# TejasPote/data_diet_distributed

Measured on AMD Instinct MI355X. Metric: examples scored/sec (whole node), EL2N+GraNd ResNet-18 CIFAR-10, 1/2/4/8 GPU, higher is better.
Workload: dtype fp32 (split MFMA: hi*hi + hi*lo + lo*hi with fp32 accumulation; EL2N forward on f16x3 halves, GraNd forward on f16x3, GraNd backward on bf16x3); 1 GPU; R18/C10 EL2N+GraNd, K checkpoints, global keep-set; arch=resnet18, input=3x32x32 cifar stem, n_examples=50000, checkpoints=10, classes=10, score_batch=128, grand_batch=1024, el2n_chunk=1024, kept=25000, select_by=el2n, pegrad_method=auto, grand_params=conv_linear, passes=sequential, lanes=3, launch_plan=full chunks + short tail, el2n_operands=f16x3

## Files before the change

data_diet_distributed_amd/csrc/dd_down.hip:

```cpp
#include "dd_mfma.h"

#include <stdlib.h>

namespace dd {
namespace down {

using namespace conv;

template <int WO, int RB, int E>
struct DCfg {
  static constexpr int SR = 2 * RB + 1;
  static constexpr int NR = E * SR;
  static constexpr int WI = 2 * WO;
  static constexpr int XS = WO * 2;
  static constexpr int PLANE = CC * XS;
  static constexpr int ROWP = 3 * 2 * PLANE + (WO == 16 ? 64 : WO == 8 ? 32 : WO == 4 ? 16 : 0);
  static constexpr int IMGP = SR * ROWP + (WO == 4 ? 240 : 0);
  static constexpr int BUF = E * IMGP;
  static constexpr int TB = E * RB * WO;
  static constexpr int TPR = WI / 8;
  static constexpr int NF8 = NR * CC * WI / 8;
  static constexpr int NST = (NF8 + 255) / 256;
  static constexpr int TPR4 = WI / 4;
  static constexpr int NF4 = NR * CC * WI / 4;
  static constexpr int NST4 = (NF4 + 255) / 256;
  static constexpr int TAILB = (NF8 % 256 != 0 || NF4 % 256 != 0) ? 6 * PLANE + 512 : 0;
  static constexpr int LDS = 2 * BUF + TAILB;
  static_assert(TB == 64, "two 32-position t tiles per workgroup");
  static_assert(WO % 4 == 0, "transposed reads take 4 consecutive columns");
  static_assert(BUF >= 4 * 4096, "the epilogue's four 4 KB transpose blocks live in a buffer");
};

struct Out {
  float* y;
  const float* bias;
  float* stats;
  int relu;
  float scale;
};

struct FwdArgs {
  const float* x;
  const __bf16* w3;
  const __bf16* ws;
  Out main, sc;
  int64_t B, n_stat;
  int cin, HO, cout, nob32;
  int gsize, tiles_per_group, n_tb, n_ob, n_tiles;
  int xcd;
  int wog;
  const float* in_scale;
  const float* in_shift;
  const float* xres;
};

constexpr int kXmNone = 0, kXmAffine = 1, kXmUnit = 3;

template <int WO, int RB, int E, bool SC, bool PT, int WA, int EPI = 0, int XM = 0,
          bool F16 = false, int PW = 0>
__global__ __launch_bounds__(256, 2) void down_fwd_kernel(const FwdArgs A) {
  using C = DCfg<WO, RB, E>;
  constexpr int NT = WA == 4 ? 2 : 1;
  constexpr bool S8 = WO >= 8;
  static_assert(!PW || (!SC && S8 && E == 1 && XM != kXmUnit && EPI == 0),
                "padded-width heads: the plain EL2N statistics launch");
  extern __shared__ __attribute__((aligned(16))) char smem[];
  const int HO = A.HO, HI = 2 * HO, cin = A.cin, cout = A.cout;
  const int64_t B = A.B;
  const int WOG = PW ? A.wog : WO, WIG = 2 * WOG;
  const int HWI = HI * WIG, HWO = HO * WOG;
  const int ntiles = A.n_tiles;

  const int tid = threadIdx.x, lane = tid & 63;
  const int wv = WA == 4 ? __builtin_amdgcn_readfirstlane(tid >> 6) : tid >> 6;
  const int wo = WA == 4 ? wv : wv & 1, wt = WA == 4 ? 0 : wv >> 1, h = lane >> 5;

  struct Tile {
    int64_t b, grp;
    int tb, y0, o_w, ob32;
  };
  auto decode = [&](int tile) {
    Tile T;
    int bid = tile;
    const int ob = bid % A.n_ob;
    bid /= A.n_ob;
    T.tb = bid % A.n_tb;
    T.b = (int64_t)(bid / A.n_tb) * E;
    T.y0 = T.tb * RB;
    T.grp = T.b / A.gsize;
    T.o_w = ob * 32 * WA + wo * 32;
    T.ob32 = T.o_w >> 5;
    return T;
  };

  const float* __restrict__ x = A.x;
  float4 ra4[S8 ? 1 : C::NST4];
  bool va4[S8 ? 1 : C::NST4];
  static_assert(256 % (C::TPR4 * CC) == 0 && 256 % (C::TPR * CC) == 0,
                "a thread's staged channel must not depend on the round");
  float xs = 1.f, xt = 0.f;
  float4 rr4[(S8 || XM != kXmUnit) ? 1 : C::NST4];
  float4 rr8[(S8 && XM == kXmUnit) ? C::NST : 1][2];
  auto load_affine = [&](const Tile& T, int c0, int tpr) {
    if constexpr (XM != kXmNone) {
      const int cg = c0 + (tid / tpr) % CC;
      const int xi = (int)(T.grp * cin) + (cg < cin ? cg : cin - 1);
      xs = A.in_scale[xi];
      xt = A.in_shift[xi];
    }
  };
  auto xform = [&](float4 v, float4 r) {
    if constexpr (XM == kXmNone) {
      return v;
    } else {
      v = make_float4(fmaf(v.x, xs, xt), fmaf(v.y, xs, xt), fmaf(v.z, xs, xt), fmaf(v.w, xs, xt));
      if constexpr (XM == kXmUnit) v = make_float4(v.x + r.x, v.y + r.y, v.z + r.z, v.w + r.w);
      return make_float4(nmax(v.x, 0.f), nmax(v.y, 0.f), nmax(v.z, 0.f), nmax(v.w, 0.f));
    }
  };
  auto load_chunk4 = [&](const Tile& T, int c0) {
#pragma unroll
    for (int k = 0; k < C::NST4; ++k) {
      const int q = tid + 256 * k;
      const int x4 = q % C::TPR4, c = (q / C::TPR4) % CC, sr = q / (C::TPR4 * CC);
      const int e = sr / C::SR, rr = sr - e * C::SR;
      const int ir = 2 * T.y0 - 1 + rr, cg = c0 + c;
      const bool ve = T.b + e < B;
      va4[k] = q < C::NF4 && ir >= 0 && ir < HI && cg < cin && ve;
      const int irc = ir < 0 ? 0 : (ir >= HI ? HI - 1 : ir);
      const int cgc = cg < cin ? cg : cin - 1;
      const int64_t bc = ve ? T.b + e : B - 1;
      const size_t ofs = ((size_t)bc * cin + cgc) * HWI + irc * C::WI + x4 * 4;
      ra4[k] = *reinterpret_cast<const float4*>(x + ofs);
      if constexpr (!S8 && XM == kXmUnit) rr4[k] = *reinterpret_cast<const float4*>(A.xres + ofs);
    }
    load_affine(T, c0, C::TPR4);
  };
  auto store_chunk4 = [&](int buf) {
    char* base0 = smem + buf * C::BUF;
#pragma unroll
    for (int k = 0; k < C::NST4; ++k) {
      const int q = tid + 256 * k;
      const bool tail = C::NF4 % 256 != 0 && k == C::NST4 - 1 && q >= C::NF4;
      const int x4 = q % C::TPR4, c = (q / C::TPR4) % CC, sr = q / (C::TPR4 * CC);
      float4 rk = make_float4(0.f, 0.f, 0.f, 0.f);
      if constexpr (!S8 && XM == kXmUnit) rk = rr4[k];
      const float4 v = keep_if(xform(ra4[k], rk), va4[k]);
      float left = lane_prev<C::TPR4>(v.w);
      if (x4 == 0) left = 0.f;
      const float f[3][2] = {{left, v.y}, {v.x, v.z}, {v.y, v.w}};
#pragma unroll
      for (int kx = 0; kx < 3; ++kx) {
        __bf16 h0, l0, h1, l1;
        split16<F16>(f[kx][0], h0, l0);
        split16<F16>(f[kx][1], h1, l1);
        const int se = sr / C::SR, rr = sr - se * C::SR;
        char* p = tail ? smem + 2 * C::BUF + (kx * 2) * C::PLANE + lane * 4
                       : base0 + se * C::IMGP + rr * C::ROWP + (kx * 2) * C::PLANE + c * C::XS +
                             x4 * 4;
        typedef __bf16 bf16x2 __attribute__((ext_vector_type(2)));
        *reinterpret_cast<bf16x2*>(p) = bf16x2{h0, h1};
        *reinterpret_cast<bf16x2*>(p + C::PLANE) = bf16x2{l0, l1};
      }
    }
  };

  float4 ra[S8 ? C::NST : 1][2];
  bool va[S8 ? C::NST : 1];
  auto load_chunk8 = [&](const Tile& T, int c0) {
#pragma unroll
    for (int k = 0; k < C::NST; ++k) {
      const int q = tid + 256 * k;
      const int x8 = q % C::TPR, c = (q / C::TPR) % CC, sr = q / (C::TPR * CC);
      const int e = sr / C::SR, rr = sr - e * C::SR;
      const int ir = 2 * T.y0 - 1 + rr, cg = c0 + c;
      const bool ve = T.b + e < B;
      va[k] = q < C::NF8 && ir >= 0 && ir < HI && cg < cin && ve && (!PW || x8 * 8 < WIG);
      const int irc = ir < 0 ? 0 : (ir >= HI ? HI - 1 : ir);
      const int cgc = cg < cin ? cg : cin - 1;
      const int64_t bc = ve ? T.b + e : B - 1;
      const int col = PW && x8 * 8 >= WIG ? 0 : x8 * 8;
      const size_t ofs = ((size_t)bc * cin + cgc) * HWI + irc * WIG + col;
      if constexpr (PW == 3) {
        float v[8];
#pragma unroll
        for (int j = 0; j < 8; ++j) v[j] = x[ofs + (col + j < WIG ? j : 0)];
        ra[k][0] = make_float4(v[0], v[1], v[2], v[3]);
        ra[k][1] = make_float4(v[4], v[5], v[6], v[7]);
      } else {
        ra[k][0] = *reinterpret_cast<const float4*>(x + ofs);
        ra[k][1] = *reinterpret_cast<const float4*>(x + ofs + (!PW || col + 4 < WIG ? 4 : 0));
      }
      if constexpr (S8 && XM == kXmUnit) {
        rr8[k][0] = *reinterpret_cast<const float4*>(A.xres + ofs);
        rr8[k][1] = *reinterpret_cast<const float4*>(A.xres + ofs + 4);
      }
    }
    load_affine(T, c0, C::TPR);
  };
  auto store_chunk8 = [&](int buf) {
    char* base0 = smem + buf * C::BUF;
#pragma unroll
    for (int k = 0; k < C::NST; ++k) {
      const int q = tid + 256 * k;
      const bool tail = C::NF8 % 256 != 0 && k == C::NST - 1 && q >= C::NF8;
      const int x8 = q % C::TPR, c = (q / C::TPR) % CC, sr = q / (C::TPR * CC);
      float4 r0 = make_float4(0.f, 0.f, 0.f, 0.f), r1 = r0;
      if constexpr (S8 && XM == kXmUnit) {
        r0 = rr8[k][0];
        r1 = rr8[k][1];
      }
      float4 v0 = keep_if(xform(ra[k][0], r0), va[k]), v1 = keep_if(xform(ra[k][1], r1), va[k]);
      if constexpr (PW != 0) {
        v0 = keep_cols(v0, WIG - x8 * 8);
        v1 = keep_cols(v1, WIG - x8 * 8 - 4);
      }
      float left = C::TPR > 1 ? lane_prev<C::TPR>(v1.w) : 0.f;
      if (x8 == 0) left = 0.f;
      const float f[9] = {left, v0.x, v0.y, v0.z, v0.w, v1.x, v1.y, v1.z, v1.w};
      __bf16 hv[9], lv[9];
#pragma unroll
      for (int i = 0; i < 9; ++i) split16<F16>(f[i], hv[i], lv[i]);
      const int se = sr / C::SR, rr = sr - se * C::SR;
#pragma unroll
      for (int kx = 0; kx < 3; ++kx) {
        char* p = tail ? smem + 2 * C::BUF + (kx * 2) * C::PLANE + lane * 8
                       : base0 + se * C::IMGP + rr * C::ROWP + (kx * 2) * C::PLANE + c * C::XS +
                             x8 * 8;
        *reinterpret_cast<bf16x4*>(p) = bf16x4{hv[kx], hv[kx + 2], hv[kx + 4], hv[kx + 6]};
        *reinterpret_cast<bf16x4*>(p + C::PLANE) = bf16x4{lv[kx], lv[kx + 2], lv[kx + 4], lv[kx + 6]};
      }
    }
  };

  auto load_chunk = [&](const Tile& T, int c0) {
    if constexpr (S8) load_chunk8(T, c0); else load_chunk4(T, c0);
  };
  auto store_chunk = [&](int buf) {
    if constexpr (S8) store_chunk8(buf); else store_chunk4(buf);
  };

  bf16x8 wa[18], wsc[2];
  const __bf16* __restrict__ w3 = A.w3;
  const __bf16* __restrict__ wsp = A.ws;
  auto load_w_taps = [&](int ob32, int kc, int tap0, int ntap) {
    const int blk = min(ob32, A.nob32 - 1);
    const __bf16* base = w3 + ((size_t)(kc * A.nob32 + blk) * 18) * 512 + lane * 8;
#pragma unroll
    for (int i = 0; i < 18; ++i)
      if (i >= 2 * tap0 && i < 2 * (tap0 + ntap))
        wa[i] = *reinterpret_cast<const bf16x8*>(base + i * 512);
  };
  auto load_w_sc = [&](int ob32, int kc) {
    if constexpr (SC) {
      const int blk = min(ob32, A.nob32 - 1);
      const __bf16* base = wsp + ((size_t)(kc * A.nob32 + blk) * 2) * 512 + lane * 8;
      wsc[0] = *reinterpret_cast<const bf16x8*>(base);
      wsc[1] = *reinterpret_cast<const bf16x8*>(base + 512);
    }
  };
  auto load_w_ordered = [&](int ob32, int kc) {
    static_for<9>([&](auto Tc) {
      load_w_taps(ob32, kc, decltype(Tc)::value, 1);
      if constexpr (decltype(Tc)::value == 4) load_w_sc(ob32, kc);
      __builtin_amdgcn_sched_barrier(0);
    });
  };

  const int q = (lane >> 2) & 3, p = lane & 3, g1 = (lane >> 4) & 1;
  int tr_off[NT];
#pragma unroll
  for (int n = 0; n < NT; ++n) {
    const int t = (wt + n) * 32 + 16 * g1 + 4 * p;
    const int e = t / (RB * WO);
    tr_off[n] = e * C::IMGP + 2 * ((t / WO) % RB) * C::ROWP + (8 * h + q) * C::XS + (t % WO) * 2;
  }

  floatx16 acc[NT], acc_s[NT];
  auto read_b = [&](const char* base, int ky, bf16x8 (&bf)[3][2]) {
#pragma unroll
    for (int kx = 0; kx < 3; ++kx) {
      const char* a = base + tr_off[0] + ky * C::ROWP + (kx * 2) * C::PLANE;
      bf[kx][0] = tr_read8(a, a + 4 * C::XS);
      bf[kx][1] = tr_read8(a + C::PLANE, a + C::PLANE + 4 * C::XS);
    }
  };
  auto mfma_row = [&](int ky, const bf16x8 (&bf)[3][2]) {
#pragma unroll
    for (int kx = 0; kx < 3; ++kx) {
      const int tap = ky * 3 + kx;
      floatx16 d = acc[0];
      d = mfma16<F16>(wa[tap * 2], bf[kx][0], d);
      d = mfma16<F16>(wa[tap * 2], bf[kx][1], d);
      d = mfma16<F16>(wa[tap * 2 + 1], bf[kx][0], d);
      acc[0] = d;
      if constexpr (SC) {
        if (ky == 1 && kx == 1) {
          floatx16 s = acc_s[0];
          s = mfma16<F16>(wsc[0], bf[1][0], s);
          s = mfma16<F16>(wsc[0], bf[1][1], s);
          s = mfma16<F16>(wsc[1], bf[1][0], s);
          acc_s[0] = s;
        }
      }
    }
  };

  auto epilogue = [&](const Tile& T, const floatx16& a, const Out& out, const int o_w,
                      char* ep_buf, const int tc, auto MAINc) {
    constexpr bool MAIN = decltype(MAINc)::value;
    const bool has_bias = EPI == 0 ? out.bias != nullptr : EPI == 2;
    const bool relu = EPI == 0 ? out.relu != 0 : (EPI == 2 && MAIN);
    const bool has_stats = EPI == 0 ? out.stats != nullptr : EPI == 1;
    float* ep = reinterpret_cast<float*>(ep_buf) + wv * 1024;
    const int tl = lane & 7, ol = lane >> 3;
#pragma unroll
    for (int r = 0; r < 16; ++r)
      ep[((r & 3) + 8 * (r >> 2) + 4 * h) * 32 + (lane & 31)] = F16 ? a[r] * out.scale : a[r];
    asm volatile("" ::: "memory");
    float4 v[4];
#pragma unroll
    for (int k = 0; k < 4; ++k)
      v[k] = *reinterpret_cast<const float4*>(ep + (8 * k + ol) * 32 + 4 * tl);
    asm volatile("" ::: "memory");
    const int tt = tc * 32 + 4 * tl;
    const int e = tt / (RB * WO);
    int t = T.y0 * WO + tt % (RB * WO);
    bool in_map = true;
    int ncol = 4;
    if constexpr (PW != 0) {
      const int rem = tt % (RB * WO), row = T.y0 + rem / WO, col = rem % WO;
      in_map = row < HO && col < WOG;
      ncol = WOG - col;
      t = in_map ? row * WOG + col : 0;
    }
    const bool ve = T.b + e < B && in_map;
    const float in_stat = (T.b + e < A.n_stat && in_map) ? 1.f : 0.f;
    const int64_t be = T.b + e < B ? T.b + e : B - 1;
    const int frag = ((int)((T.b - T.grp * A.gsize) / E) * A.n_tb + T.tb) * 2 + tc;
    float* const sp = has_stats ? out.stats + (((size_t)T.grp * cout + o_w + ol) *
                                               A.tiles_per_group + frag) * 2 : nullptr;
#pragma unroll
    for (int k = 0; k < 4; ++k) {
      const int o = o_w + 8 * k + ol;
      const float bia = has_bias ? out.bias[o < cout ? o : cout - 1] : 0.f;
      float f[4] = {v[k].x, v[k].y, v[k].z, v[k].w};
      float s_ = 0.f, q_ = 0.f;
#pragma unroll
      for (int j = 0; j < 4; ++j) {
        float u = f[j] + bia;
        if (relu) u = nmax(u, 0.f);
        f[j] = u;
        const float us = (PW >= 2 && j >= ncol) ? 0.f : u * in_stat;
        s_ += us;
        q_ += us * us;
      }
      if constexpr (PW >= 2) {
        if (ve && o < cout) {
#pragma unroll
          for (int j = 0; j < 4; ++j)
            if (j < ncol) out.y[((size_t)be * cout + o) * HWO + t + j] = f[j];
        }
      } else if (ve && o < cout) {
        store_out4(out.y + ((size_t)be * cout + o) * HWO + t, f[0], f[1], f[2], f[3]);
      }
      if (has_stats) {
        s_ = sum8(s_);
        q_ = sum8(q_);
        if (tl == 0 && o < cout)
          *reinterpret_cast<float2*>(sp + k * 16 * A.tiles_per_group) = make_float2(s_, q_);
      }
    }
    asm volatile("" ::: "memory");
  };

  const int nchunks = (cin + CC - 1) / CC;
  int tile = A.xcd >= (PT ? 2 : 1) ? (int)xcd_order(blockIdx.x, gridDim.x) : (int)blockIdx.x;
  Tile T = decode(tile);
  load_chunk(T, 0);
  __builtin_amdgcn_sched_barrier(0);
  load_w_ordered(T.ob32, 0);
  store_chunk(0);
  __syncthreads();
  int g = 0;
  for (;;) {
    const int tile_n = tile + (int)gridDim.x;
    const bool has_next = PT && tile_n < ntiles;
#pragma unroll
    for (int n = 0; n < NT; ++n) acc[n] = acc_s[n] = floatx16{0};
    auto chunk4 = [&](const Tile& Tp, int kn, bool wload) {
      const int cur = g & 1;
      load_chunk(Tp, kn * CC);
      __builtin_amdgcn_sched_barrier(0);
      const char* base = smem + cur * C::BUF;
      bf16x8 bb[NT][2];
      auto rb = [&](int tap, int n) {
        const char* a = base + tr_off[n] + (tap / 3) * C::ROWP + ((tap % 3) * 2) * C::PLANE;
        bb[n][0] = tr_read8(a, a + 4 * C::XS);
        bb[n][1] = tr_read8(a + C::PLANE, a + C::PLANE + 4 * C::XS);
      };
#pragma unroll
      for (int n = 0; n < NT; ++n) rb(0, n);
      static_for<9>([&](auto Tc) {
        constexpr int t = decltype(Tc)::value;
#pragma unroll
        for (int n = 0; n < NT; ++n) {
          floatx16 d = acc[n];
          d = mfma16<F16>(wa[t * 2], bb[n][0], d);
          d = mfma16<F16>(wa[t * 2], bb[n][1], d);
          d = mfma16<F16>(wa[t * 2 + 1], bb[n][0], d);
          acc[n] = d;
          if constexpr (SC && t == 4) {
            floatx16 s_ = acc_s[n];
            s_ = mfma16<F16>(wsc[0], bb[n][0], s_);
            s_ = mfma16<F16>(wsc[0], bb[n][1], s_);
            s_ = mfma16<F16>(wsc[1], bb[n][0], s_);
            acc_s[n] = s_;
          }
          if constexpr (t + 1 < 9) rb(t + 1, n);
        }
        if (wload) {
          load_w_taps(Tp.ob32, kn, t, 1);
          if constexpr (t == 4) load_w_sc(Tp.ob32, kn);
        }
        if constexpr (t == 6) store_chunk(cur ^ 1);
        __builtin_amdgcn_sched_barrier(0);
      });
      __syncthreads();
      ++g;
    };
    auto chunk = [&](const Tile& Tp, int kn, bool wload) {
      if constexpr (WA == 4) {
        chunk4(Tp, kn, wload);
        return;
      }
      const int cur = g & 1;
      load_chunk(Tp, kn * CC);
      const char* base = smem + cur * C::BUF;
      bf16x8 b0[3][2], b1[3][2];
      read_b(base, 0, b0);
      __builtin_amdgcn_sched_barrier(0);
      read_b(base, 1, b1);
      mfma_row(0, b0);
      if (wload) load_w_taps(Tp.ob32, kn, 0, 3);
#pragma unroll
      for (int i = 0; i < 3; ++i) {
        __builtin_amdgcn_sched_group_barrier(0x008, 1, 0);
        __builtin_amdgcn_sched_group_barrier(0x100, 2, 0);
        __builtin_amdgcn_sched_group_barrier(0x008, 1, 0);
        __builtin_amdgcn_sched_group_barrier(0x100, 2, 0);
        __builtin_amdgcn_sched_group_barrier(0x020, 2, 0);
        __builtin_amdgcn_sched_group_barrier(0x008, 1, 0);
      }
      __builtin_amdgcn_sched_barrier(0);
      read_b(base, 2, b0);
      mfma_row(1, b1);
      if (wload) {
        load_w_taps(Tp.ob32, kn, 3, 3);
        load_w_sc(Tp.ob32, kn);
      }
#pragma unroll
      for (int i = 0; i < 3; ++i) {
        __builtin_amdgcn_sched_group_barrier(0x008, 1, 1);
        __builtin_amdgcn_sched_group_barrier(0x100, 2, 1);
        __builtin_amdgcn_sched_group_barrier(0x008, 1, 1);
        __builtin_amdgcn_sched_group_barrier(0x100, 2, 1);
        __builtin_amdgcn_sched_group_barrier(0x020, 2, 1);
        __builtin_amdgcn_sched_group_barrier(0x008, 1, 1);
      }
      __builtin_amdgcn_sched_barrier(0);
      mfma_row(2, b0);
      store_chunk(cur ^ 1);
      if (wload) load_w_taps(Tp.ob32, kn, 6, 3);
#pragma unroll
      for (int i = 0; i < 9; ++i) {
        __builtin_amdgcn_sched_group_barrier(0x008, 1, 2);
        __builtin_amdgcn_sched_group_barrier(0x002, 5, 2);
        __builtin_amdgcn_sched_group_barrier(0x080, 1, 2);
      }
      __builtin_amdgcn_sched_barrier(0);
      __syncthreads();
      ++g;
    };
    for (int kc = 0; kc + 1 < nchunks; ++kc) chunk(T, kc + 1, true);
    {
      const Tile Tn = has_next ? decode(tile_n) : T;
      chunk(Tn, has_next ? 0 : nchunks - 1, false);
    }
    char* ep_buf = smem + ((g - 1) & 1) * C::BUF;
#pragma unroll
    for (int n = 0; n < NT; ++n) {
      epilogue(T, acc[n], A.main, T.o_w, ep_buf, wt + n, std::true_type{});
      if constexpr (SC) epilogue(T, acc_s[n], A.sc, T.o_w, ep_buf, wt + n, std::false_type{});
    }
    if constexpr (!PT) break;
    __syncthreads();
    const int tile_w = has_next ? tile_n : tile;
    T = decode(tile_w);
    load_w_ordered(T.ob32, 0);
    if (!has_next) break;
    tile = tile_n;
  }
}

template <int WO, int RB, int E, bool SC>
struct UCfg {
  static constexpr int NRH = E * (RB + 1);
  static constexpr int NRZ = E * RB;
  static constexpr int XS = WO * 2;
  static constexpr int PLANE = CC * XS;
  static constexpr int PADR = WO == 16 ? 128 : WO == 8 ? 64 : WO == 4 ? 32 : 0;
  static constexpr int ROWP = 2 * 2 * PLANE + PADR;
  static constexpr int IMGP = (RB + 1) * ROWP + (WO == 4 ? 224 : 0);
  static constexpr int ROWPZ = 2 * PLANE + PADR;
  static constexpr int IMGPZ = RB * ROWPZ;
  static constexpr int HBUF = E * IMGP;
  static constexpr int ZBUF = SC ? E * IMGPZ : 0;
  static constexpr int BUF = HBUF + ZBUF;
  static constexpr int TB = E * RB * WO;
  static constexpr int TPR = WO / 4;
  static constexpr int NF4H = NRH * CC * WO / 4;
  static constexpr int NF4Z = NRZ * CC * WO / 4;
  static constexpr int NSTH = (NF4H + 255) / 256;
  static constexpr int NSTZ = (NF4Z + 255) / 256;
  static constexpr int TAILB = (NF4H % 256 != 0 || NF4Z % 256 != 0) ? 4 * PLANE + 512 : 0;
  static constexpr int LDS = 2 * BUF + TAILB;
};

struct BwdArgs {
  const float* dh;
  const float* dz;
  const __bf16* w3t;
  const __bf16* w1t;
  const float* mask;
  const uint32_t* mask_bits;
  float* dx;
  int64_t B;
  int cin, cout, HO, nob32;
  int n_tb, n_ob;
  int xcd;
};

template <int WO, int RB, int E, bool SC>
__global__ __launch_bounds__(256, 2) void down_bwd_kernel(const BwdArgs A) {
  using C = UCfg<WO, RB, E, SC>;
  static_assert(C::TB == 64, "two 32-position t tiles per workgroup");
  extern __shared__ __attribute__((aligned(16))) char smem[];
  const int HO = A.HO, HI = 2 * HO, WI = 2 * WO, cin = A.cin, cout = A.cout;
  const int64_t B = A.B;
  const int HWO = HO * WO;
  int bid = blockIdx.x;
  const int ob = bid % A.n_ob;
  bid /= A.n_ob;
  const int tb = bid % A.n_tb;
  const int64_t b = (int64_t)(bid / A.n_tb) * E;
  const int i0 = tb * RB;

  const int tid = threadIdx.x, lane = tid & 63, wv = tid >> 6;
  const int wc = wv & 1, wt = wv >> 1, h = lane >> 5;
  const int c_w = ob * 64 + wc * 32;
  const int ob32 = min(c_w >> 5, A.nob32 - 1);

  float4 rh[C::NSTH], rz[C::NSTZ];
  bool vh[C::NSTH], vz[C::NSTZ];
  auto load_chunk = [&](int o0) {
#pragma unroll
    for (int k = 0; k < C::NSTH; ++k) {
      const int q = tid + 256 * k;
      const int x4 = q % C::TPR, c = (q / C::TPR) % CC, sr = q / (C::TPR * CC);
      const int e = sr / (RB + 1), rr = sr - e * (RB + 1);
      const int ir = i0 + rr, og = o0 + c;
      const bool ve = b + e < B;
// ... 357 lines not shown
          const int c = c_w + (r & 3) + 8 * (r >> 2) + 4 * h;
          const size_t off =
              (((size_t)be * cin + (c < cin ? c : cin - 1)) * HI + 2 * i + py) * WI + 2 * j;
          const float2 m2 = *reinterpret_cast<const float2*>(A.mask + off);
          mk[r] = (m2.x > 0.f ? 1u : 0u) | (m2.y > 0.f ? 2u : 0u);
        }
      } else {
#pragma unroll
        for (int r = 0; r < 16; ++r) mk[r] = 3u;
      }
#pragma unroll
      for (int r = 0; r < 16; ++r) {
        const int c = c_w + (r & 3) + 8 * (r >> 2) + 4 * h;
        const size_t off =
            (((size_t)be * cin + (c < cin ? c : cin - 1)) * HI + 2 * i + py) * WI + 2 * j;
        float2 v = make_float2(acc[py * 2][n][r], acc[py * 2 + 1][n][r]);
        if (!(mk[r] & 1u)) v.x = 0.f;
        if (!(mk[r] & 2u)) v.y = 0.f;
        if (ve && c < cin) *reinterpret_cast<float2*>(A.dx + off) = v;
      }
    }
  }
}

__global__ void pack1x1_kernel(const float* __restrict__ w, int cout, int cin, int tflip, int op,
                               int cp, int f16, float scale, __bf16* __restrict__ out) {
  const int nob32 = op / 32, nkc = cp / CC;
  const int total = nkc * nob32 * 2 * 512;
  for (int i = blockIdx.x * blockDim.x + threadIdx.x; i < total; i += gridDim.x * blockDim.x) {
    const int j = i & 7, lane = (i >> 3) & 63;
    int r = i >> 9;
    const int pr = r & 1;
    r >>= 1;
    const int blk = r % nob32, kc = r / nob32;
    const int o = blk * 32 + (lane & 31), c = kc * CC + 8 * (lane >> 5) + j;
    const int no = tflip ? cin : cout, nc = tflip ? cout : cin;
    float v = 0.f;
    if (o < no && c < nc) v = tflip ? w[(size_t)c * cin + o] : w[(size_t)o * cin + c];
    v *= scale;
    __bf16 hi, lo;
    if (f16)
      split16<true>(v, hi, lo);
    else
      split16<false>(v, hi, lo);
    out[i] = pr == 0 ? hi : lo;
  }
}

template <int WO, int RB, int E, bool SC, int WA, int EPI = 0, int XM = 0, bool F16 = false>
static int launch_fwd(FwdArgs a, hipStream_t st) {
  using C = DCfg<WO, RB, E>;
  static bool attr = false;
  if (!attr) {
    (void)hipFuncSetAttribute(
        reinterpret_cast<const void*>(&down_fwd_kernel<WO, RB, E, SC, false, WA, EPI, XM, F16>),
        hipFuncAttributeMaxDynamicSharedMemorySize, C::LDS);
    (void)hipFuncSetAttribute(
        reinterpret_cast<const void*>(&down_fwd_kernel<WO, RB, E, SC, true, WA, EPI, XM, F16>),
        hipFuncAttributeMaxDynamicSharedMemorySize, C::LDS);
    attr = true;
  }
  DD_REQUIRE(a.HO % RB == 0, "dd_down_forward: HO must be a multiple of the row block");
  DD_REQUIRE(a.gsize % E == 0, "dd_down_forward: group_size %d must be a multiple of %d",
             a.gsize, E);
  a.n_tb = a.HO / RB;
  a.n_ob = (int)ceil_div(a.cout, 32 * WA);
  a.tiles_per_group = (a.gsize / E) * a.n_tb * 2;
  const int64_t ntiles = ceil_div(a.B, E) * a.n_tb * a.n_ob;
  DD_REQUIRE(ntiles < (1ll << 31), "dd_down_forward: too many tiles");
  a.n_tiles = (int)ntiles;
  const bool pt = a.cin <= 64;
  const int64_t cap = pt ? 2ll * device_cus() : ntiles;
  const int64_t grid = ntiles < cap ? ntiles : cap;
  if (pt)
    down_fwd_kernel<WO, RB, E, SC, true, WA, EPI, XM, F16>
        <<<(unsigned)grid, 256, C::LDS, st>>>(a);
  else
    down_fwd_kernel<WO, RB, E, SC, false, WA, EPI, XM, F16>
        <<<(unsigned)grid, 256, C::LDS, st>>>(a);
  DD_CHECK_LAUNCH("dd_down_forward");
  return DD_OK;
}

template <int WO, int RB, int PW, int XM, bool F16>
static int launch_fwd_pw(FwdArgs a, hipStream_t st) {
  using C = DCfg<WO, RB, 1>;
  constexpr auto K = &down_fwd_kernel<WO, RB, 1, false, false, 4, 0, XM, F16, PW>;
  static bool attr = false;
  if (!attr) {
    (void)hipFuncSetAttribute(reinterpret_cast<const void*>(K),
                              hipFuncAttributeMaxDynamicSharedMemorySize, C::LDS);
    attr = true;
  }
  a.n_tb = (a.HO + RB - 1) / RB;
  a.n_ob = (int)ceil_div(a.cout, 128);
  a.tiles_per_group = a.gsize * a.n_tb * 2;
  const int64_t ntiles = a.B * a.n_tb * a.n_ob;
  DD_REQUIRE(ntiles < (1ll << 31), "dd_down_forward: too many tiles");
  a.n_tiles = (int)ntiles;
  K<<<(unsigned)ntiles, 256, C::LDS, st>>>(a);
  DD_CHECK_LAUNCH("dd_down_forward");
  return DD_OK;
}

static int fwd_epi(const Out& m, const Out& s) {
  static const int f = env_int("DD_DOWN_EPI", 1);
  if (f == 0 || !s.y) return 0;
  if (!m.bias && !m.relu && m.stats && !s.bias && !s.relu && s.stats) return 1;
  if (m.bias && m.relu && !m.stats && s.bias && !s.relu && !s.stats) return 2;
  return 0;
}
static int fwd_wa(int cout) {
  static const int f = env_int("DD_DOWN_WA", 4);
  return f == 4 && conv::pad_to(cout, 64) % 128 == 0 ? 4 : 2;
}

template <int WO, int RB, int E, bool SC>
static int launch_bwd(BwdArgs a, hipStream_t st) {
  using C = UCfg<WO, RB, E, SC>;
  static bool attr = false;
  if (!attr) {
    (void)hipFuncSetAttribute(reinterpret_cast<const void*>(&down_bwd_kernel<WO, RB, E, SC>),
                              hipFuncAttributeMaxDynamicSharedMemorySize, C::LDS);
    attr = true;
  }
  DD_REQUIRE(a.HO % RB == 0, "dd_down_backward: HO must be a multiple of the row block");
  a.n_tb = a.HO / RB;
  a.n_ob = (int)ceil_div(a.cin, 64);
  const int64_t grid = ceil_div(a.B, E) * a.n_tb * a.n_ob;
  DD_REQUIRE(grid < (1ll << 31), "dd_down_backward: grid too large");
  down_bwd_kernel<WO, RB, E, SC><<<(unsigned)grid, 256, C::LDS, st>>>(a);
  DD_CHECK_LAUNCH("dd_down_backward");
  return DD_OK;
}

template <int WO, int RB, int E, bool SC>
static int launch_bwd2(BwdArgs a, hipStream_t st) {
  using C = UCfg<WO, RB, E, SC>;
  static bool attr = false;
  if (!attr) {
    (void)hipFuncSetAttribute(reinterpret_cast<const void*>(&down_bwd2_kernel<WO, RB, E, SC>),
                              hipFuncAttributeMaxDynamicSharedMemorySize, C::LDS);
    attr = true;
  }
  static_assert(2 * C::LDS <= 160 * 1024, "two workgroups per CU");
  DD_REQUIRE(a.HO % RB == 0, "dd_down_backward: HO must be a multiple of the row block");
  a.n_tb = a.HO / RB;
  a.n_ob = (int)ceil_div(a.cin, 64);
  const int64_t grid = ceil_div(a.B, E) * a.n_tb * a.n_ob;
  DD_REQUIRE(grid < (1ll << 31), "dd_down_backward: grid too large");
  down_bwd2_kernel<WO, RB, E, SC><<<(unsigned)grid, 256, C::LDS, st>>>(a);
  DD_CHECK_LAUNCH("dd_down_backward");
  return DD_OK;
}

static bool bwd2() {
  static const int f = env_int("DD_DOWN_BWD", 2);
  return f == 2;
}

static int pw_geometry(int ho, int wo, int* rb, int* pw) {
  if (env_int("DD_DOWN_PW", 1) == 0 || ho <= 0) return 0;
  if (wo > 16 && wo <= 32 && wo % 4 == 0) { *rb = 2; *pw = 1; return 32; }
  if (wo > 8 && wo <= 16 && wo % 2 == 0) { *rb = 4; *pw = 2; return 16; }
  if (wo > 4 && wo <= 8) { *rb = 8; *pw = 3; return 8; }
  return 0;
}

static bool geometry(int ho, int wo, int* rb, int* e) {
  if (wo == 32 && ho % 2 == 0) { *rb = 2; *e = 1; return true; }
  if (wo == 16 && ho % 4 == 0) { *rb = 4; *e = 1; return true; }
  if (wo == 8 && ho == 8) { *rb = 8; *e = 1; return true; }
  if (wo == 4 && ho == 4) { *rb = 4; *e = 4; return true; }
  return false;
}

}
}

using namespace dd;

extern "C" {

size_t dd_conv1x1_pack_bytes(int32_t out_channels, int32_t in_channels) {
  if (out_channels <= 0 || in_channels <= 0) return 0;
  return (size_t)2 * conv::pad_to(out_channels, 64) * conv::pad_to(in_channels, 2 * conv::CC) *
         sizeof(__bf16);
}

int dd_conv1x1_pack(const float* w, int32_t cout, int32_t cin, int32_t transpose,
                    int32_t operands, float scale, void* packed, void* stream) {
  clear_error();
  DD_REQUIRE(w && packed && cout > 0 && cin > 0, "dd_conv1x1_pack: bad arguments");
  DD_REQUIRE(operands == DD_OPERANDS_BF16X3 || operands == DD_OPERANDS_F16X3,
             "dd_conv1x1_pack: operands must be DD_OPERANDS_BF16X3 or DD_OPERANDS_F16X3");
  DD_REQUIRE(operand_scale_ok(operands, scale),
             "dd_conv1x1_pack: scale must be 1 (bf16 operands) or a power of two (fp16)");
  const int no = transpose ? cin : cout, nc = transpose ? cout : cin;
  const int op = conv::pad_to(no, 64), cp = conv::pad_to(nc, 2 * conv::CC);
  const int total = 2 * op * cp;
  down::pack1x1_kernel<<<(unsigned)std::min<int64_t>(ceil_div(total, 256), 4096), 256, 0,
                         as_stream(stream)>>>(w, cout, cin, transpose, op, cp,
                                              operands == DD_OPERANDS_F16X3, scale,
                                              static_cast<__bf16*>(packed));
  DD_CHECK_LAUNCH("dd_conv1x1_pack");
  return DD_OK;
}

int dd_down_tiles_per_group(int32_t ho, int32_t wo, int32_t group_size) {
  int rb, e, pw;
  if (group_size <= 0) return -1;
  if (!down::geometry(ho, wo, &rb, &e)) {
    if (!down::pw_geometry(ho, wo, &rb, &pw)) return -1;
    return group_size * ((ho + rb - 1) / rb) * 2;
  }
  if (group_size % e) return -1;
  return (group_size / e) * (ho / rb) * 2;
}

int dd_down_padded_supported(int32_t ho, int32_t wo, int32_t cin, int32_t cout,
                             int32_t group_size) {
  int rb, e, pw;
  if (ho <= 0 || wo <= 0 || cin <= 64 || cout <= 0 || group_size <= 0 ||
      down::geometry(ho, wo, &rb, &e) || !down::pw_geometry(ho, wo, &rb, &pw))
    return 0;
  return down::fwd_wa(cout) == 4 && (int64_t)cin * 4 * ho * wo < (1ll << 31) ? 1 : 0;
}

static int down_forward_impl(const float* x, int64_t B, int32_t cin, int32_t ho, int32_t wo,
                             const void* packed3x3, const void* packed1x1, int32_t cout,
                             const float* bias, int32_t relu, float* stats, float* y,
                             const float* bias_sc, int32_t relu_sc, float* stats_sc,
                             float* y_sc, int32_t group_size, int64_t n_stat,
                             const float* in_scale, const float* in_shift, const float* xres,
                             int32_t operands, float acc_scale, float acc_scale_sc,
                             void* stream) {
  DD_REQUIRE(B >= 0 && cin > 0 && cout > 0 && ho > 0, "dd_down_forward: bad sizes");
  DD_REQUIRE(operands == DD_OPERANDS_BF16X3 || operands == DD_OPERANDS_F16X3,
             "dd_down_forward: operands must be DD_OPERANDS_BF16X3 or DD_OPERANDS_F16X3");
  DD_REQUIRE(operand_scale_ok(operands, acc_scale) && operand_scale_ok(operands, acc_scale_sc),
             "dd_down_forward: acc_scale must be 1 (bf16 operands) or a power of two (fp16)");
  if (B == 0) return DD_OK;
  DD_REQUIRE(x && packed3x3 && y, "dd_down_forward: null buffer");
  DD_REQUIRE(!packed1x1 == !y_sc, "dd_down_forward: shortcut pack and output go together");
  DD_REQUIRE(cin > conv::CC / 3, "dd_down_forward: cin %d <= %d is packed in the stem layout",
             cin, conv::CC / 3);
  DD_REQUIRE((int64_t)cin * 4 * ho * wo < (1ll << 31), "dd_down_forward: tensor too large");
  const bool grouped = stats || stats_sc;
  DD_REQUIRE(!grouped || group_size > 0, "dd_down_forward: group_size must be positive");
  int rb, e, pw = 0, pw_w = 0;
  if (!down::geometry(ho, wo, &rb, &e)) {
    if (stats && !packed1x1 && !bias && !relu && !xres &&
        dd_down_padded_supported(ho, wo, cin, cout, group_size))
      pw_w = down::pw_geometry(ho, wo, &rb, &pw);
    if (!pw_w) {
      set_error("dd_down_forward: unsupported output shape %dx%d (32 wide with even HO, 16 wide "
                "with HO %% 4 == 0, 8x8 or 4x4; other widths up to 32 for the statistics "
                "launch without a shortcut, cin > 64, cout padded to 128)", ho, wo);
      return DD_EINVAL;
    }
    e = 1;
  }
  down::FwdArgs a{};
  a.x = x;
  a.w3 = static_cast<const __bf16*>(packed3x3);
  a.ws = static_cast<const __bf16*>(packed1x1);
  a.main = down::Out{y, bias, stats, relu, acc_scale};
  a.sc = down::Out{y_sc, bias_sc, stats_sc, relu_sc, acc_scale_sc};
  a.B = B;
  a.n_stat = grouped ? std::min<int64_t>(std::max<int64_t>(n_stat, 0), B) : 0;
  a.cin = cin;
  a.HO = ho;
  a.cout = cout;
  a.nob32 = conv::pad_to(cout, 64) / 32;
  a.gsize = grouped ? group_size : (int)(std::min<int64_t>(B + e, 1 << 30) / e * e);
  static const int xcd = env_int("DD_DOWN_XCD", 2);
  a.xcd = xcd;
  hipStream_t st = as_stream(stream);
  const bool sc = packed1x1 != nullptr;
  a.in_scale = in_scale;
  a.in_shift = in_shift;
  a.xres = xres;
  a.wog = wo;
  if (pw_w) {
    const bool f16 = operands == DD_OPERANDS_F16X3, xf = in_scale != nullptr;
#define DD_DOWN_PWL(WO_, RB_, PW_)                                                              \
    if (pw_w == WO_ && pw == PW_)                                                               \
      return f16 ? (xf ? down::launch_fwd_pw<WO_, RB_, PW_, down::kXmAffine, true>(a, st)       \
                       : down::launch_fwd_pw<WO_, RB_, PW_, down::kXmNone, true>(a, st))        \
                 : (xf ? down::launch_fwd_pw<WO_, RB_, PW_, down::kXmAffine, false>(a, st)      \
                       : down::launch_fwd_pw<WO_, RB_, PW_, down::kXmNone, false>(a, st));
    DD_DOWN_PWL(32, 2, 1)
    DD_DOWN_PWL(16, 4, 2)
    DD_DOWN_PWL(8, 8, 3)
#undef DD_DOWN_PWL
    set_error("dd_down_forward: no padded-width head for width %d", wo);
    return DD_EINVAL;
  }
  if (operands == DD_OPERANDS_F16X3) {
    const int wa = down::fwd_wa(cout);
    const int epi = down::fwd_epi(a.main, a.sc);
    DD_REQUIRE(!xres || (sc && epi == 1),
               "dd_down_forward_unit_input: the unit form needs the fused shortcut and "
               "statistics on both outputs");
    DD_REQUIRE(!in_scale || xres || !sc,
               "dd_down_forward_unit_input: BN + ReLU staging without a shortcut only");
#define DD_DOWN_F(WO_, RB_, E_, WA_)                                                          \
    if (xres) return down::launch_fwd<WO_, RB_, E_, true, WA_, 1, down::kXmUnit, true>(a, st); \
    if (in_scale) return down::launch_fwd<WO_, RB_, E_, false, WA_, 0, down::kXmAffine, true>(a, st); \
    if (sc && epi == 1) return down::launch_fwd<WO_, RB_, E_, true, WA_, 1, 0, true>(a, st); \
    if (sc && epi == 2) return down::launch_fwd<WO_, RB_, E_, true, WA_, 2, 0, true>(a, st); \
    if (sc) return down::launch_fwd<WO_, RB_, E_, true, WA_, 0, 0, true>(a, st);           \
    return down::launch_fwd<WO_, RB_, E_, false, WA_, 0, 0, true>(a, st);
#define DD_DOWN_FW(WO_, RB_, E_) \
    if (wa == 4) { DD_DOWN_F(WO_, RB_, E_, 4) } else { DD_DOWN_F(WO_, RB_, E_, 2) }
    if (wo == 32) { DD_DOWN_FW(32, 2, 1) }
    if (wo == 16) { DD_DOWN_FW(16, 4, 1) }
    if (wo == 8) { DD_DOWN_FW(8, 8, 1) }
    DD_DOWN_FW(4, 4, 4)
#undef DD_DOWN_FW
#undef DD_DOWN_F
  }
  if (in_scale) {
    const int wa = down::fwd_wa(cout);
#define DD_DOWN_X(WO_, RB_, E_)                                                          \
    if (xres) {                                                                          \
      DD_REQUIRE(sc && down::fwd_epi(a.main, a.sc) == 1,                                 \
                 "dd_down_forward_unit_input: the unit form needs the fused shortcut and " \
                 "statistics on both outputs");                                          \
      return wa == 4 ? down::launch_fwd<WO_, RB_, E_, true, 4, 1, down::kXmUnit>(a, st) \
                     : down::launch_fwd<WO_, RB_, E_, true, 2, 1, down::kXmUnit>(a, st); \
    }                                                                                    \
    DD_REQUIRE(!sc, "dd_down_forward_unit_input: BN + ReLU staging without a shortcut only"); \
    return wa == 4 ? down::launch_fwd<WO_, RB_, E_, false, 4, 0, down::kXmAffine>(a, st) \
                   : down::launch_fwd<WO_, RB_, E_, false, 2, 0, down::kXmAffine>(a, st);
    if (wo == 32) { DD_DOWN_X(32, 2, 1) }
    if (wo == 16) { DD_DOWN_X(16, 4, 1) }
    if (wo == 8) { DD_DOWN_X(8, 8, 1) }
    DD_DOWN_X(4, 4, 4)
#undef DD_DOWN_X
  }
  const int wa = down::fwd_wa(cout);
  const int epi = down::fwd_epi(a.main, a.sc);
#define DD_DOWN_SC(WO_, RB_, E_, WA_)                                                  \
  (epi == 1   ? down::launch_fwd<WO_, RB_, E_, true, WA_, 1>(a, st)                \
   : epi == 2 ? down::launch_fwd<WO_, RB_, E_, true, WA_, 2>(a, st)                \
              : down::launch_fwd<WO_, RB_, E_, true, WA_, 0>(a, st))
#define DD_DOWN(WO_, RB_, E_)                                                    \
  return wa == 4 ? (sc ? DD_DOWN_SC(WO_, RB_, E_, 4)                             \
                       : down::launch_fwd<WO_, RB_, E_, false, 4>(a, st))        \
                 : (sc ? DD_DOWN_SC(WO_, RB_, E_, 2)                             \
                       : down::launch_fwd<WO_, RB_, E_, false, 2>(a, st))
  if (wo == 32) DD_DOWN(32, 2, 1);
  if (wo == 16) DD_DOWN(16, 4, 1);
  if (wo == 8) DD_DOWN(8, 8, 1);
  DD_DOWN(4, 4, 4);
#undef DD_DOWN
#undef DD_DOWN_SC
}

int dd_down_forward(const float* x, int64_t B, int32_t cin, int32_t ho, int32_t wo,
                    const void* packed3x3, const void* packed1x1, int32_t cout,
                    const float* bias, int32_t relu, float* stats, float* y,
                    const float* bias_sc, int32_t relu_sc, float* stats_sc, float* y_sc,
                    int32_t group_size, int64_t n_stat, int32_t operands, float acc_scale,
                    float acc_scale_sc, void* stream) {
  clear_error();
  return down_forward_impl(x, B, cin, ho, wo, packed3x3, packed1x1, cout, bias, relu, stats, y,
                           bias_sc, relu_sc, stats_sc, y_sc, group_size, n_stat, nullptr,
                           nullptr, nullptr, operands, acc_scale, acc_scale_sc, stream);
}

int dd_down_forward_unit_input(const float* y_prev, const float* in_scale,
                               const float* in_shift, const float* res, int64_t B, int32_t cin,
                               int32_t ho, int32_t wo, const void* packed3x3,
                               const void* packed1x1, int32_t cout, float* stats, float* y,
                               float* stats_sc, float* y_sc, int32_t group_size,
                               int64_t n_stat, int32_t operands, float acc_scale,
                               float acc_scale_sc, void* stream) {
  clear_error();
  DD_REQUIRE(B >= 0, "dd_down_forward_unit_input: bad sizes");
// ... 69 lines not shown
```

Measured before the change: 8530 examples/s.

## Add 128-position single-buffer tile variant for fused-shortcut downsample forward

Adds a T128 variant of the downsample conv forward kernel in which each workgroup covers four 32-position t fragments (128 positions) instead of two, on the fused-shortcut scoring launches at widths 16 and 8. The variant uses one LDS buffer instead of two, staggers input staging in rounds with loads overlapped against stores, and keeps a rotating three-tap weight register window that prefetches taps ahead. The aim is to reuse each weight load across more output positions and to cut LDS and register pressure. The cost is that the single buffer serialises staging and compute with an extra barrier per chunk. It is enabled by default through an env flag.

```diff
diff --git a/data_diet_distributed_amd/csrc/dd_down.hip b/data_diet_distributed_amd/csrc/dd_down.hip
--- a/data_diet_distributed_amd/csrc/dd_down.hip
+++ b/data_diet_distributed_amd/csrc/dd_down.hip
@@ -1,13 +1,14 @@
 #include "dd_mfma.h"
 
 #include <stdlib.h>
+#include <string.h>
 
 namespace dd {
 namespace down {
 
 using namespace conv;
 
-template <int WO, int RB, int E>
+template <int WO, int RB, int E, int NBUF = 2>
 struct DCfg {
   static constexpr int SR = 2 * RB + 1;
   static constexpr int NR = E * SR;
@@ -25,8 +26,9 @@
   static constexpr int NF4 = NR * CC * WI / 4;
   static constexpr int NST4 = (NF4 + 255) / 256;
   static constexpr int TAILB = (NF8 % 256 != 0 || NF4 % 256 != 0) ? 6 * PLANE + 512 : 0;
-  static constexpr int LDS = 2 * BUF + TAILB;
-  static_assert(TB == 64, "two 32-position t tiles per workgroup");
+  static constexpr int LDS = NBUF * BUF + TAILB;
+  static constexpr int NFRAG = TB / 32;
+  static_assert(TB == 64 || TB == 128, "two or four 32-position t tiles per workgroup");
   static_assert(WO % 4 == 0, "transposed reads take 4 consecutive columns");
   static_assert(BUF >= 4 * 4096, "the epilogue's four 4 KB transpose blocks live in a buffer");
 };
@@ -57,10 +59,14 @@
 constexpr int kXmNone = 0, kXmAffine = 1, kXmUnit = 3;
 
 template <int WO, int RB, int E, bool SC, bool PT, int WA, int EPI = 0, int XM = 0,
-          bool F16 = false, int PW = 0>
+          bool F16 = false, int PW = 0, bool T128 = false>
 __global__ __launch_bounds__(256, 2) void down_fwd_kernel(const FwdArgs A) {
-  using C = DCfg<WO, RB, E>;
-  constexpr int NT = WA == 4 ? 2 : 1;
+  constexpr int NBUF = T128 ? 1 : 2;
+  using C = DCfg<WO, RB, E, NBUF>;
+  constexpr int NT = WA == 4 ? C::NFRAG : 1;
+  static_assert(!T128 || !PT, "the 128-position tile runs one tile per workgroup");
+  static_assert(!T128 ? C::TB == 64 : (C::TB == 128 && WA == 4 && SC && !PW && EPI != 0),
+                "128-position tiles: four waves along o, the fused-shortcut scoring launches");
   constexpr bool S8 = WO >= 8;
   static_assert(!PW || (!SC && S8 && E == 1 && XM != kXmUnit && EPI == 0),
                 "padded-width heads: the plain EL2N statistics launch");
@@ -118,9 +124,10 @@
       return make_float4(nmax(v.x, 0.f), nmax(v.y, 0.f), nmax(v.z, 0.f), nmax(v.w, 0.f));
     }
   };
-  auto load_chunk4 = [&](const Tile& T, int c0) {
+  auto load_chunk4 = [&](const Tile& T, int c0, int k0, int k1) {
 #pragma unroll
     for (int k = 0; k < C::NST4; ++k) {
+      if (k < k0 || k >= k1) continue;
       const int q = tid + 256 * k;
       const int x4 = q % C::TPR4, c = (q / C::TPR4) % CC, sr = q / (C::TPR4 * CC);
       const int e = sr / C::SR, rr = sr - e * C::SR;
@@ -134,12 +141,13 @@
       ra4[k] = *reinterpret_cast<const float4*>(x + ofs);
       if constexpr (!S8 && XM == kXmUnit) rr4[k] = *reinterpret_cast<const float4*>(A.xres + ofs);
     }
-    load_affine(T, c0, C::TPR4);
-  };
-  auto store_chunk4 = [&](int buf) {
+    if (k0 == 0) load_affine(T, c0, C::TPR4);
+  };
+  auto store_chunk4 = [&](int buf, int k0, int k1) {
     char* base0 = smem + buf * C::BUF;
 #pragma unroll
     for (int k = 0; k < C::NST4; ++k) {
+      if (k < k0 || k >= k1) continue;
       const int q = tid + 256 * k;
       const bool tail = C::NF4 % 256 != 0 && k == C::NST4 - 1 && q >= C::NF4;
       const int x4 = q % C::TPR4, c = (q / C::TPR4) % CC, sr = q / (C::TPR4 * CC);
@@ -155,7 +163,7 @@
         split16<F16>(f[kx][0], h0, l0);
         split16<F16>(f[kx][1], h1, l1);
         const int se = sr / C::SR, rr = sr - se * C::SR;
-        char* p = tail ? smem + 2 * C::BUF + (kx * 2) * C::PLANE + lane * 4
+        char* p = tail ? smem + NBUF * C::BUF + (kx * 2) * C::PLANE + lane * 4
                        : base0 + se * C::IMGP + rr * C::ROWP + (kx * 2) * C::PLANE + c * C::XS +
                              x4 * 4;
         typedef __bf16 bf16x2 __attribute__((ext_vector_type(2)));
@@ -167,9 +175,10 @@
 
   float4 ra[S8 ? C::NST : 1][2];
   bool va[S8 ? C::NST : 1];
-  auto load_chunk8 = [&](const Tile& T, int c0) {
+  auto load_chunk8 = [&](const Tile& T, int c0, int k0, int k1) {
 #pragma unroll
     for (int k = 0; k < C::NST; ++k) {
+      if (k < k0 || k >= k1) continue;
       const int q = tid + 256 * k;
       const int x8 = q % C::TPR, c = (q / C::TPR) % CC, sr = q / (C::TPR * CC);
       const int e = sr / C::SR, rr = sr - e * C::SR;
@@ -196,12 +205,13 @@
         rr8[k][1] = *reinterpret_cast<const float4*>(A.xres + ofs + 4);
       }
     }
-    load_affine(T, c0, C::TPR);
-  };
-  auto store_chunk8 = [&](int buf) {
+    if (k0 == 0) load_affine(T, c0, C::TPR);
+  };
+  auto store_chunk8 = [&](int buf, int k0, int k1) {
     char* base0 = smem + buf * C::BUF;
 #pragma unroll
     for (int k = 0; k < C::NST; ++k) {
+      if (k < k0 || k >= k1) continue;
       const int q = tid + 256 * k;
       const bool tail = C::NF8 % 256 != 0 && k == C::NST - 1 && q >= C::NF8;
       const int x8 = q % C::TPR, c = (q / C::TPR) % CC, sr = q / (C::TPR * CC);
@@ -224,7 +234,7 @@
       const int se = sr / C::SR, rr = sr - se * C::SR;
 #pragma unroll
       for (int kx = 0; kx < 3; ++kx) {
-        char* p = tail ? smem + 2 * C::BUF + (kx * 2) * C::PLANE + lane * 8
+        char* p = tail ? smem + NBUF * C::BUF + (kx * 2) * C::PLANE + lane * 8
                        : base0 + se * C::IMGP + rr * C::ROWP + (kx * 2) * C::PLANE + c * C::XS +
                              x8 * 8;
         *reinterpret_cast<bf16x4*>(p) = bf16x4{hv[kx], hv[kx + 2], hv[kx + 4], hv[kx + 6]};
@@ -233,14 +243,28 @@
     }
   };
 
-  auto load_chunk = [&](const Tile& T, int c0) {
-    if constexpr (S8) load_chunk8(T, c0); else load_chunk4(T, c0);
-  };
-  auto store_chunk = [&](int buf) {
-    if constexpr (S8) store_chunk8(buf); else store_chunk4(buf);
-  };
-
-  bf16x8 wa[18], wsc[2];
+  constexpr int NRND = S8 ? C::NST : C::NST4;
+  auto load_rounds = [&](const Tile& T, int c0, int k0, int k1) {
+    if constexpr (S8) load_chunk8(T, c0, k0, k1); else load_chunk4(T, c0, k0, k1);
+  };
+  auto store_rounds = [&](int buf, int k0, int k1) {
+    if constexpr (S8) store_chunk8(buf, k0, k1); else store_chunk4(buf, k0, k1);
+  };
+  auto load_chunk = [&](const Tile& T, int c0) { load_rounds(T, c0, 0, NRND); };
+  auto store_chunk = [&](int buf) { store_rounds(buf, 0, NRND); };
+  auto stage_chunk = [&](const Tile& T, int c0, int buf) {
+    constexpr int SD = S8 ? (XM == kXmUnit ? 2 : 3) : (XM == kXmUnit ? 3 : 5);
+    load_rounds(T, c0, 0, SD);
+    static_for<NRND>([&](auto Kc) {
+      constexpr int k = decltype(Kc)::value;
+      __builtin_amdgcn_sched_barrier(0);
+      store_rounds(buf, k, k + 1);
+      if constexpr (k + SD < NRND) load_rounds(T, c0, k + SD, k + SD + 1);
+    });
+  };
+
+  constexpr int NWS = T128 ? 3 : 9;
+  bf16x8 wa[2 * NWS], wsc[2];
   const __bf16* __restrict__ w3 = A.w3;
   const __bf16* __restrict__ wsp = A.ws;
   auto load_w_taps = [&](int ob32, int kc, int tap0, int ntap) {
@@ -249,7 +273,7 @@
 #pragma unroll
     for (int i = 0; i < 18; ++i)
       if (i >= 2 * tap0 && i < 2 * (tap0 + ntap))
-        wa[i] = *reinterpret_cast<const bf16x8*>(base + i * 512);
+        wa[(i / 2 % NWS) * 2 + (i & 1)] = *reinterpret_cast<const bf16x8*>(base + i * 512);
   };
   auto load_w_sc = [&](int ob32, int kc) {
     if constexpr (SC) {
@@ -260,9 +284,9 @@
     }
   };
   auto load_w_ordered = [&](int ob32, int kc) {
-    static_for<9>([&](auto Tc) {
+    static_for<NWS>([&](auto Tc) {
       load_w_taps(ob32, kc, decltype(Tc)::value, 1);
-      if constexpr (decltype(Tc)::value == 4) load_w_sc(ob32, kc);
+      if constexpr (decltype(Tc)::value == (T128 ? 2 : 4)) load_w_sc(ob32, kc);
       __builtin_amdgcn_sched_barrier(0);
     });
   };
@@ -337,7 +361,9 @@
     const bool ve = T.b + e < B && in_map;
     const float in_stat = (T.b + e < A.n_stat && in_map) ? 1.f : 0.f;
     const int64_t be = T.b + e < B ? T.b + e : B - 1;
-    const int frag = ((int)((T.b - T.grp * A.gsize) / E) * A.n_tb + T.tb) * 2 + tc;
+    const int frag = ((int)((T.b - T.grp * A.gsize) / E) * A.n_tb + T.tb) * C::NFRAG + tc;
+    constexpr int E64 = C::TB == 128 && E > 1 ? E / 2 : E;
+    const bool frag_live = C::TB == 64 || T.b + e / E64 * E64 < B;
     float* const sp = has_stats ? out.stats + (((size_t)T.grp * cout + o_w + ol) *
                                                A.tiles_per_group + frag) * 2 : nullptr;
 #pragma unroll
@@ -367,7 +393,7 @@
       if (has_stats) {
         s_ = sum8(s_);
         q_ = sum8(q_);
-        if (tl == 0 && o < cout)
+        if (tl == 0 && o < cout && frag_live)
           *reinterpret_cast<float2*>(sp + k * 16 * A.tiles_per_group) = make_float2(s_, q_);
       }
     }
@@ -377,10 +403,15 @@
   const int nchunks = (cin + CC - 1) / CC;
   int tile = A.xcd >= (PT ? 2 : 1) ? (int)xcd_order(blockIdx.x, gridDim.x) : (int)blockIdx.x;
   Tile T = decode(tile);
-  load_chunk(T, 0);
-  __builtin_amdgcn_sched_barrier(0);
-  load_w_ordered(T.ob32, 0);
-  store_chunk(0);
+  if constexpr (T128) {
+    load_w_ordered(T.ob32, 0);
+    stage_chunk(T, 0, 0);
+  } else {
+    load_chunk(T, 0);
+    __builtin_amdgcn_sched_barrier(0);
+    load_w_ordered(T.ob32, 0);
+    store_chunk(0);
+  }
   __syncthreads();
   int g = 0;
   for (;;) {
@@ -388,9 +419,10 @@
     const bool has_next = PT && tile_n < ntiles;
 #pragma unroll
     for (int n = 0; n < NT; ++n) acc[n] = acc_s[n] = floatx16{0};
-    auto chunk4 = [&](const Tile& Tp, int kn, bool wload) {
-      const int cur = g & 1;
-      load_chunk(Tp, kn * CC);
+    auto chunk4 = [&](const Tile& Tp, int kn, int kcur, bool wload, auto LASTc) {
+      constexpr bool LAST = decltype(LASTc)::value;
+      const int cur = T128 ? 0 : g & 1;
+      if constexpr (!T128) load_chunk(Tp, kn * CC);
       __builtin_amdgcn_sched_barrier(0);
       const char* base = smem + cur * C::BUF;
       bf16x8 bb[NT][2];
@@ -406,9 +438,9 @@
 #pragma unroll
         for (int n = 0; n < NT; ++n) {
           floatx16 d = acc[n];
-          d = mfma16<F16>(wa[t * 2], bb[n][0], d);
-          d = mfma16<F16>(wa[t * 2], bb[n][1], d);
-          d = mfma16<F16>(wa[t * 2 + 1], bb[n][0], d);
+          d = mfma16<F16>(wa[(t % NWS) * 2], bb[n][0], d);
+          d = mfma16<F16>(wa[(t % NWS) * 2], bb[n][1], d);
+          d = mfma16<F16>(wa[(t % NWS) * 2 + 1], bb[n][0], d);
           acc[n] = d;
           if constexpr (SC && t == 4) {
             floatx16 s_ = acc_s[n];
@@ -419,19 +451,34 @@
           }
           if constexpr (t + 1 < 9) rb(t + 1, n);
         }
-        if (wload) {
-          load_w_taps(Tp.ob32, kn, t, 1);
-          if constexpr (t == 4) load_w_sc(Tp.ob32, kn);
+        if constexpr (T128) {
+          if constexpr (t + 3 < 9) {
+            load_w_taps(T.ob32, kcur, t + 3, 1);
+          } else if (wload) {
+            load_w_taps(Tp.ob32, kn, t + 3 - 9, 1);
+          }
+          if constexpr (t == 4)
+            if (wload) load_w_sc(Tp.ob32, kn);
+        } else {
+          if (wload) {
+            load_w_taps(Tp.ob32, kn, t, 1);
+            if constexpr (t == 4) load_w_sc(Tp.ob32, kn);
+          }
+          if constexpr (t == 6) store_chunk(cur ^ 1);
         }
-        if constexpr (t == 6) store_chunk(cur ^ 1);
         __builtin_amdgcn_sched_barrier(0);
       });
       __syncthreads();
+      if constexpr (T128 && !LAST) {
+        __builtin_amdgcn_sched_barrier(0);
+        stage_chunk(Tp, kn * CC, 0);
+        __syncthreads();
+      }
       ++g;
     };
-    auto chunk = [&](const Tile& Tp, int kn, bool wload) {
+    auto chunk = [&](const Tile& Tp, int kn, int kcur, bool wload, auto LASTc) {
       if constexpr (WA == 4) {
-        chunk4(Tp, kn, wload);
+        chunk4(Tp, kn, kcur, wload, LASTc);
         return;
       }
       const int cur = g & 1;
@@ -482,12 +529,12 @@
       __syncthreads();
       ++g;
     };
-    for (int kc = 0; kc + 1 < nchunks; ++kc) chunk(T, kc + 1, true);
+    for (int kc = 0; kc + 1 < nchunks; ++kc) chunk(T, kc + 1, kc, true, std::false_type{});
     {
       const Tile Tn = has_next ? decode(tile_n) : T;
-      chunk(Tn, has_next ? 0 : nchunks - 1, false);
-    }
-    char* ep_buf = smem + ((g - 1) & 1) * C::BUF;
+      chunk(Tn, has_next ? 0 : nchunks - 1, nchunks - 1, false, std::true_type{});
+    }
+    char* ep_buf = smem + (T128 ? 0 : (g - 1) & 1) * C::BUF;
 #pragma unroll
     for (int n = 0; n < NT; ++n) {
       epilogue(T, acc[n], A.main, T.o_w, ep_buf, wt + n, std::true_type{});
@@ -1011,6 +1058,28 @@
   return DD_OK;
 }
 
+template <int WO, int RB, int E, int EPI, int XM, bool F16>
+static int launch_fwd128(FwdArgs a, hipStream_t st) {
+  using C = DCfg<WO, RB, E, 1>;
+  static_assert(2 * C::LDS <= 160 * 1024, "two workgroups per CU");
+  constexpr auto K = &down_fwd_kernel<WO, RB, E, true, false, 4, EPI, XM, F16, 0, true>;
+  static bool attr = false;
+  if (!attr) {
+    (void)hipFuncSetAttribute(reinterpret_cast<const void*>(K),
+                              hipFuncAttributeMaxDynamicSharedMemorySize, C::LDS);
+    attr = true;
+  }
+  a.n_tb = a.HO / RB;
+  a.n_ob = (int)ceil_div(a.cout, 128);
+  a.tiles_per_group = (a.gsize / E) * a.n_tb * C::NFRAG;
+  const int64_t ntiles = ceil_div(a.B, E) * a.n_tb * a.n_ob;
+  DD_REQUIRE(ntiles < (1ll << 31), "dd_down_forward: too many tiles");
+  a.n_tiles = (int)ntiles;
+  K<<<(unsigned)ntiles, 256, C::LDS, st>>>(a);
+  DD_CHECK_LAUNCH("dd_down_forward");
+  return DD_OK;
+}
+
 template <int WO, int RB, int PW, int XM, bool F16>
 static int launch_fwd_pw(FwdArgs a, hipStream_t st) {
   using C = DCfg<WO, RB, 1>;
@@ -1094,6 +1163,16 @@
   if (wo > 8 && wo <= 16 && wo % 2 == 0) { *rb = 4; *pw = 2; return 16; }
   if (wo > 4 && wo <= 8) { *rb = 8; *pw = 3; return 8; }
   return 0;
+}
+
+static bool geometry128(int ho, int wo, int* rb, int* e) {
+  if (wo == 16 && ho % 8 == 0) { *rb = 8; *e = 1; return true; }
+  if (wo == 8 && ho == 8) { *rb = 8; *e = 2; return true; }
+  return false;
+}
+static bool fwd_t128() {
+  const char* e = env_str("DD_DOWN_T128");
+  return !e || !*e || !strcmp(e, "auto") || atoi(e) != 0;
 }
 
 static bool geometry(int ho, int wo, int* rb, int* e) {
@@ -1226,6 +1305,24 @@
     set_error("dd_down_forward: no padded-width head for width %d", wo);
     return DD_EINVAL;
   }
+  {
+    int rb2, e2;
+    const int epi = down::fwd_epi(a.main, a.sc);
+    const bool f16 = operands == DD_OPERANDS_F16X3;
+    if (sc && (epi == 2 ? !in_scale : (epi == 1 && f16 && !in_scale == !xres)) &&
+        down::fwd_wa(cout) == 4 && down::geometry128(ho, wo, &rb2, &e2) &&
+        (!grouped || group_size % e2 == 0) && down::fwd_t128()) {
+      if (!grouped) a.gsize = (int)(std::min<int64_t>(B + e2, 1 << 30) / e2 * e2);
+#define DD_DOWN_T(WO_, RB_, E_)                                                            \
+      if (xres) return down::launch_fwd128<WO_, RB_, E_, 1, down::kXmUnit, true>(a, st);   \
+      if (epi == 1) return down::launch_fwd128<WO_, RB_, E_, 1, 0, true>(a, st);           \
+      return f16 ? down::launch_fwd128<WO_, RB_, E_, 2, 0, true>(a, st)                    \
+                 : down::launch_fwd128<WO_, RB_, E_, 2, 0, false>(a, st);
+      if (wo == 16) { DD_DOWN_T(16, 8, 1) }
+      DD_DOWN_T(8, 8, 2)
+#undef DD_DOWN_T
+    }
+  }
   if (operands == DD_OPERANDS_F16X3) {
     const int wa = down::fwd_wa(cout);
     const int epi = down::fwd_epi(a.main, a.sc);
```

New measurement: 8605 examples/s (median of 6 runs). About the same (+0.9%).
